# hliangzhao/torch-on-k8s

Hardware: AMD Instinct MI355X
Metric: tokens_per_s (higher is better)
Workload: dtype bf16; 1 GPU; model=llama3-8b, global_batch=8, seq_len=4096, parallelism=dp1, attn_impl=hip

## Files before the change

torch_on_k8s_amd/ops/csrc/attention.hip:

```cpp
#include "common.h"

namespace {

using bf16x8v = __attribute__((ext_vector_type(8))) __bf16;
using f32x4 = __attribute__((ext_vector_type(4))) float;

constexpr int BN = 64;
constexpr int NW = 8;
constexpr int NTHREADS = NW * WAVE;
constexpr int BM = NW * 16;
constexpr float NEG_INF = -INFINITY;

DEVINL int swz_off(int row, int row_bytes, int byte_in_row) {
  return (row * row_bytes + byte_in_row) ^ ((row & 15) << 4);
}

DEVINL bf16x8v as_frag(uint4 raw) {
  union { uint4 u; bf16x8v f; } c;
  c.u = raw;
  return c.f;
}

template <int D, int NTH = NTHREADS>
struct TileStage {
// ... 20 lines not shown
      const int vi = threadIdx.x + i * NTH;
      const int row = vi / VPR, cv = vi % VPR;
      *(uint4*)(lds + swz_off(row, D * 2, cv * 16)) = vals[i];
    }
  }

};

template <int D, int NTH = NTHREADS>
struct TileStageT {
  static constexpr int VPR = 64 / 8;
  static constexpr int VPT = D * VPR / NTH;
  uint4 vals[VPT];

  DEVINL void issue(const bf16_t* plane, int col0, long S_pad) {
#pragma unroll
    for (int i = 0; i < VPT; ++i) {
      const int vi = threadIdx.x + i * NTH;
      const int row = vi / VPR, cv = vi % VPR;
      vals[i] = *(const uint4*)(plane + (long)row * S_pad + col0 + cv * 8);
    }
  }

  DEVINL void write(char* lds) const {
#pragma unroll
    for (int i = 0; i < VPT; ++i) {
      const int vi = threadIdx.x + i * NTH;
      const int row = vi / VPR, cv = vi % VPR;
      *(uint4*)(lds + swz_off(row, 128, cv * 16)) = vals[i];
    }
  }
};

template <int RB>
DEVINL bf16x8v read_bfrag(const char* lds, int row, int col_elem) {
  return as_frag(*(const uint4*)(lds + swz_off(row, RB, col_elem * 2)));
}

template <int D>
DEVINL void load_afrags(bf16x8v* frag, const bf16_t* src, long row,
                        long row_limit, long tok_stride, int lane) {
  constexpr int DC = D / 32;
#pragma unroll
  for (int c = 0; c < DC; ++c) {
    uint4 raw = {0, 0, 0, 0};
    if (row < row_limit)
      raw = *(const uint4*)(src + row * tok_stride + c * 32 + (lane >> 4) * 8);
    frag[c] = as_frag(raw);
  }
}

using f32x16 = __attribute__((ext_vector_type(16))) float;

DEVINL uint32_t pack_bf16(float lo, float hi) {
  return (uint32_t)f2bfbits(lo) | ((uint32_t)f2bfbits(hi) << 16);
}

template <int D, bool CAUSAL>
__global__ __launch_bounds__(NTHREADS) void attn_fwd_kernel_v3(
    const bf16_t* __restrict__ q, const bf16_t* __restrict__ k,
    const bf16_t* __restrict__ vt, bf16_t* __restrict__ o,
    float* __restrict__ lse, int B, int S, int Hq, int Hkv, int S_pad,
    float scale) {
  constexpr int QC = D / 16;
  constexpr int DT = D / 32;
  constexpr int BM3 = NW * 32;
  constexpr int KB = BN * D * 2;
  __shared__ __attribute__((aligned(16))) char smem[2 * (2 * KB)];

  const int lane = threadIdx.x & 63;
  const int hi = lane >> 5;
  const int wid = threadIdx.x >> 6;
  const int m0 = blockIdx.x * BM3;
  const int m0w = m0 + wid * 32;
  const int hq = blockIdx.y;
  const int b = blockIdx.z;
  const int hkv = hq / (Hq / Hkv);

  const long q_tok = (long)Hq * D, kv_tok = (long)Hkv * D;
  const bf16_t* qp = q + ((long)b * S * q_tok) + (long)hq * D;
  const bf16_t* kp = k + ((long)b * S * kv_tok) + (long)hkv * D;
  const bf16_t* vtp = vt + ((long)b * Hkv + hkv) * D * (long)S_pad;
  bf16_t* op = o + ((long)b * S * q_tok) + (long)hq * D;
  float* lsep = lse + ((long)b * Hq + hq) * S;

  const int qrow = m0w + (lane & 31);
  bf16x8v q_reg[QC];
#pragma unroll
  for (int c = 0; c < QC; ++c) {
    uint4 raw = {0, 0, 0, 0};
    if (qrow < S)
      raw = *(const uint4*)(qp + (long)qrow * q_tok + c * 16 + hi * 8);
    q_reg[c] = as_frag(raw);
  }

  f32x16 o_acc[DT];
#pragma unroll
  for (int t = 0; t < DT; ++t)
#pragma unroll
    for (int r = 0; r < 16; ++r) o_acc[t][r] = 0.f;
  float m_run = NEG_INF, l_run = 0.f;

  TileStage<D> k_st;
  TileStageT<D> v_st;
  const int n_end = CAUSAL ? min(S, m0 + BM3) : S;
  k_st.issue(kp, 0, S, kv_tok);
  v_st.issue(vtp, 0, S_pad);
  k_st.write_rm(smem);
// ... 97 lines not shown
              pack_bf16(st[ks][2], st[ks][3]),
              pack_bf16(st[ks][6], st[ks][7]), false, false);
          f0.w[0] = sA[0]; f0.w[1] = sB[0]; f0.w[2] = sA[1]; f0.w[3] = sB[1];
        }
        {
          auto sC = __builtin_amdgcn_permlane32_swap(
              pack_bf16(st[ks][8], st[ks][9]),
              pack_bf16(st[ks][12], st[ks][13]), false, false);
          auto sD = __builtin_amdgcn_permlane32_swap(
              pack_bf16(st[ks][10], st[ks][11]),
              pack_bf16(st[ks][14], st[ks][15]), false, false);
          f1.w[0] = sC[0]; f1.w[1] = sD[0]; f1.w[2] = sC[1]; f1.w[3] = sD[1];
        }
        pa[2 * ks] = f0.f;
        pa[2 * ks + 1] = f1.f;
      }

      __builtin_amdgcn_s_setprio(1);
#pragma unroll
      for (int ks = 0; ks < 4; ++ks)
#pragma unroll
        for (int t = 0; t < DT; ++t) {
          bf16x8v vb = read_bfrag<128>(
              vt_lds, t * 32 + (lane & 31), ks * 16 + hi * 8);
          o_acc[t] = __builtin_amdgcn_mfma_f32_32x32x16_bf16(
              pa[ks], vb, o_acc[t], 0, 0, 0);
        }
      __builtin_amdgcn_s_setprio(0);
    }
    if (more) {
      char* nk = smem + (cur ^ 1) * (2 * KB);
      k_st.write_rm(nk);
      v_st.write(nk + KB);
    }
    __syncthreads();
    cur ^= 1;
  }

#pragma unroll
  for (int r = 0; r < 16; ++r) {
    const int rowidx = (r & 3) + 8 * (r >> 2) + 4 * hi;
    const float lv = __shfl(l_run, rowidx, 64);
    const float inv_l = (lv > 0.f) ? 1.f / lv : 0.f;
    const int row = m0w + rowidx;
    if (row >= S) continue;
#pragma unroll
    for (int t = 0; t < DT; ++t) {
      const int col = t * 32 + (lane & 31);
      op[(long)row * q_tok + col] = f2bf(o_acc[t][r] * inv_l);
    }
  }
  if (hi == 0 && qrow < S)
    lsep[qrow] = (l_run > 0.f) ? m_run + __logf(l_run) : NEG_INF;
}

constexpr int PRE_ROWS = 64;

template <int D>
__global__ __launch_bounds__(256) void attn_bwd_pre_kernel(
    const bf16_t* __restrict__ dout, const bf16_t* __restrict__ o,
    const float* __restrict__ lse, float* __restrict__ dsum,
    float* __restrict__ rc, int Hq, int S, int S_pad, float sqrt_d) {
  constexpr int GL = D / 8;
  constexpr int RPI = WAVE / GL;
  constexpr int NP = 16 / RPI;
  const int lane = threadIdx.x & 63;
  const int wid = threadIdx.x >> 6;
  const int grp = lane / GL, gl = lane % GL;
  const int h = blockIdx.y;
  const long b = blockIdx.z;
  const int s0 = blockIdx.x * PRE_ROWS + wid * 16;
  const long tok = (long)Hq * D;
  const bf16_t* dp = dout + (b * S) * tok + (long)h * D + gl * 8;
  const bf16_t* op = o + (b * S) * tok + (long)h * D + gl * 8;

  uint4 av[NP], bv[NP];
#pragma unroll
  for (int p = 0; p < NP; ++p) {
    const int s = s0 + p * RPI + grp;
    av[p] = bv[p] = uint4{0, 0, 0, 0};
    if (s < S) {
      av[p] = *(const uint4*)(dp + (long)s * tok);
      bv[p] = *(const uint4*)(op + (long)s * tok);
    }
  }
  float mine = 0.f;
#pragma unroll
  for (int p = 0; p < NP; ++p) {
    const uint16_t* ah = (const uint16_t*)&av[p];
    const uint16_t* bh = (const uint16_t*)&bv[p];
    float acc = 0.f;
#pragma unroll
    for (int j = 0; j < 8; ++j)
      acc = fmaf(bfbits2f(ah[j]), bfbits2f(bh[j]), acc);
#pragma unroll
    for (int off = GL / 2; off > 0; off >>= 1)
      acc += __shfl_xor(acc, off, WAVE);
#pragma unroll
    for (int g = 0; g < RPI; ++g) {
      const float vg = __shfl(acc, g * GL, WAVE);
      if (lane == p * RPI + g) mine = vg;
    }
  }
  if (lane < 16) {
    const int s = s0 + lane;
    if (s < S) dsum[(b * Hq + h) * S + s] = mine;
    if (s < S_pad) {
      float* r = rc + (b * Hq + h) * 2 * S_pad;
      const float l = (s < S) ? lse[(b * Hq + h) * S + s] : NEG_INF;
      r[s] = (l == NEG_INF) ? -1e30f : -l * sqrt_d;
      r[S_pad + s] = (s < S) ? -mine : 0.f;
    }
  }
}

DEVINL void repack_pa(const f32x16& pt, bf16x8v& pa0, bf16x8v& pa1) {
  union { uint32_t w[4]; bf16x8v f; } f0, f1;
  auto sA = __builtin_amdgcn_permlane32_swap(
      pack_bf16(pt[0], pt[1]), pack_bf16(pt[4], pt[5]), false, false);
  auto sB = __builtin_amdgcn_permlane32_swap(
      pack_bf16(pt[2], pt[3]), pack_bf16(pt[6], pt[7]), false, false);
  f0.w[0] = sA[0]; f0.w[1] = sB[0]; f0.w[2] = sA[1]; f0.w[3] = sB[1];
  auto sC = __builtin_amdgcn_permlane32_swap(
      pack_bf16(pt[8], pt[9]), pack_bf16(pt[12], pt[13]), false, false);
  auto sD = __builtin_amdgcn_permlane32_swap(
      pack_bf16(pt[10], pt[11]), pack_bf16(pt[14], pt[15]), false, false);
  f1.w[0] = sC[0]; f1.w[1] = sD[0]; f1.w[2] = sC[1]; f1.w[3] = sD[1];
  pa0 = f0.f;
  pa1 = f1.f;
}

template <int D, bool CAUSAL>
__global__ __launch_bounds__(NTHREADS) void attn_bwd_dv_kernel(
    const bf16_t* __restrict__ q, const bf16_t* __restrict__ k,
    const bf16_t* __restrict__ dot_t, const bf16_t* __restrict__ dout,
    const float* __restrict__ lse, const float* __restrict__ dsum,
    bf16_t* __restrict__ dv, int B, int S, int Hq, int Hkv, int S_pad,
    float scale) {
  constexpr int QC = D / 16;
  constexpr int DT = D / 32;
  constexpr int NTH = NTHREADS;
  constexpr int BNK = NW * 32;
  constexpr int KB = BN * D * 2;
  __shared__ __attribute__((aligned(16))) char smem[2 * (2 * KB)];

  const int lane = threadIdx.x & 63;
  const int hi = lane >> 5;
  const int wid = threadIdx.x >> 6;
  const int n0 = blockIdx.x * BNK;
  const int n0w = n0 + wid * 32;
  const int hkv = blockIdx.y;
  const int b = blockIdx.z;
  const int rep = Hq / Hkv;

  const long q_tok = (long)Hq * D, kv_tok = (long)Hkv * D;
  const bf16_t* kp = k + ((long)b * S * kv_tok) + (long)hkv * D;
  bf16_t* dvp = dv + ((long)b * S * kv_tok) + (long)hkv * D;

  const int kvrow = n0w + (lane & 31);
  bf16x8v k_reg[QC];
#pragma unroll
  for (int c = 0; c < QC; ++c) {
    uint4 kr = {0, 0, 0, 0};
    if (kvrow < S)
      kr = *(const uint4*)(kp + (long)kvrow * kv_tok + c * 16 + hi * 8);
    k_reg[c] = as_frag(kr);
  }

  f32x16 dv_acc[DT];
#pragma unroll
  for (int t = 0; t < DT; ++t)
#pragma unroll
    for (int r = 0; r < 16; ++r) dv_acc[t][r] = 0.f;

  const int m_start = CAUSAL ? (n0 / BN) * BN : 0;
  const long dplane = (long)D * S_pad;
  TileStage<D, NTH> q_st;
  TileStageT<D, NTH> do_st;
  const bf16_t* dot0 = dot_t + ((long)b * Hq + hkv * rep) * dplane;
  q_st.issue(q + ((long)b * S * q_tok) + (long)(hkv * rep) * D, m_start, S,
             q_tok);
  do_st.issue(dot0, m_start, S_pad);
// ... 437 lines not shown
  constexpr int STB = DkdvStage<D>::BYTES;
  __shared__ __attribute__((aligned(16))) char smem[2 * STB + BNK * D * 2];
  char* v_lds = smem + 2 * STB;

  const int lane = threadIdx.x & 63;
  const int hi = lane >> 5;
  const int wid = threadIdx.x >> 6;
  const int n0 = blockIdx.x * BNK;
  const int n0w = n0 + wid * 64;
  const int hkv = blockIdx.y;
  const int b = blockIdx.z;
  const int rep = Hq / Hkv;

  const long q_tok = (long)Hq * D, kv_tok = (long)Hkv * D;
  const bf16_t* kp = k + ((long)b * S * kv_tok) + (long)hkv * D;
  const bf16_t* vp = v + ((long)b * S * kv_tok) + (long)hkv * D;

  bf16x8v k_reg[2][QC];
#pragma unroll
  for (int hh = 0; hh < 2; ++hh) {
    const int kvrow = n0w + hh * 32 + (lane & 31);
#pragma unroll
    for (int c = 0; c < QC; ++c) {
      uint4 kr = {0, 0, 0, 0};
      if (kvrow < S)
        kr = *(const uint4*)(kp + (long)kvrow * kv_tok + c * 16 + hi * 8);
      k_reg[hh][c] = as_frag(kr);
    }
  }
  {
    constexpr int VPR = D / 8;
#pragma unroll 4
    for (int vi = threadIdx.x; vi < BNK * VPR; vi += NTH_KV) {
      const int row = vi / VPR, cv = vi % VPR;
      uint4 val = {0, 0, 0, 0};
      if (n0 + row < S)
        val = *(const uint4*)(vp + (long)(n0 + row) * kv_tok + cv * 8);
      *(uint4*)(v_lds + swz_off(row, D * 2, cv * 16)) = val;
    }
  }

  f32x16 dk_acc[2][DT], dv_acc[2][DT];
#pragma unroll
  for (int hh = 0; hh < 2; ++hh)
#pragma unroll
    for (int t = 0; t < DT; ++t)
#pragma unroll
      for (int r = 0; r < 16; ++r) {
        dk_acc[hh][t][r] = 0.f;
        dv_acc[hh][t][r] = 0.f;
      }

  const int m_start = CAUSAL ? n0 : 0;
  const float c2 = 1.4426950408889634f * scale;
  const long plane = (long)D * S_pad;
  const long head0 = (long)b * Hq + hkv * rep;
  const bf16_t* qh = q + ((long)b * S * q_tok) + (long)(hkv * rep) * D;
  const bf16_t* doh = dout + ((long)b * S * q_tok) + (long)(hkv * rep) * D;

  DkdvStage<D> stg;
  stg.init(S_pad);
  stg.issue(qh, doh, q_t + head0 * plane, dot_t + head0 * plane,
            rc + head0 * 2 * S_pad, m_start, S, q_tok, S_pad, smem);
  stg.finish();
  __syncthreads();
  int cur = 0;

  for (int g = 0; g < rep; ++g) {
    for (int m0 = m_start; m0 < S; m0 += QROWS) {
      const char* st = smem + cur * STB;
      char* nst = smem + (cur ^ 1) * STB;
      int gn = g, mn = m0 + QROWS;
      if (mn >= S) {
        gn = g + 1;
        mn = m_start;
      }
      const bool more = gn < rep;
      const bool live0 = n0w < S && (!CAUSAL || m0 + QROWS > n0w);
      const bool live1 =
          n0w + 32 < S && (!CAUSAL || m0 + QROWS > n0w + 32);

      if (more)
        stg.issue(qh + (long)gn * D, doh + (long)gn * D,
                  q_t + (head0 + gn) * plane, dot_t + (head0 + gn) * plane,
                  rc + (head0 + gn) * 2 * S_pad, mn, S, q_tok, S_pad, nst);
      f32x16 sv[2], dpv[2];
      if (live1) {
        dkdv_tile_sdp<D, 2>(st, v_lds, k_reg, sv, dpv, wid * 64, lane, hi);
        dkdv_tile_acc<D, CAUSAL, 2>(st, sv, dpv, dk_acc, dv_acc, m0, n0w, S,
                                    lane, hi, c2);
      } else if (live0) {
        dkdv_tile_sdp<D, 1>(st, v_lds, k_reg, sv, dpv, wid * 64, lane, hi);
        dkdv_tile_acc<D, CAUSAL, 1>(st, sv, dpv, dk_acc, dv_acc, m0, n0w, S,
                                    lane, hi, c2);
      }
      if (more) stg.finish();
      __syncthreads();
      cur ^= 1;
    }
  }

  bf16_t* dkp = dk + ((long)b * S * kv_tok) + (long)hkv * D;
  bf16_t* dvp = dv + ((long)b * S * kv_tok) + (long)hkv * D;
#pragma unroll
  for (int hh = 0; hh < 2; ++hh)
#pragma unroll
    for (int r = 0; r < 16; ++r) {
// ... 5 lines not shown
        dkp[off] = f2bf(dk_acc[hh][t][r] * scale);
        dvp[off] = f2bf(dv_acc[hh][t][r]);
      }
    }
}

template <int D, bool CAUSAL>
__global__ __launch_bounds__(NTHREADS) void attn_bwd_dq_kernel(
    const bf16_t* __restrict__ q, const bf16_t* __restrict__ k,
    const bf16_t* __restrict__ v, const bf16_t* __restrict__ dout,
    const bf16_t* __restrict__ k_t, const float* __restrict__ lse,
    const float* __restrict__ dsum, bf16_t* __restrict__ dq, int B, int S,
    int Hq, int Hkv, int S_pad, float scale) {
  constexpr int QC = D / 16;
  constexpr int DT = D / 32;
  constexpr int BM3 = NW * 32;
  constexpr int KB = BN * D * 2;
  __shared__ __attribute__((aligned(16))) char smem[2 * (3 * KB)];

  const int lane = threadIdx.x & 63;
  const int hi = lane >> 5;
  const int wid = threadIdx.x >> 6;
  const int m0 =
      (CAUSAL ? (int)(gridDim.x - 1 - blockIdx.x) : (int)blockIdx.x) * BM3;
  const int m0w = m0 + wid * 32;
  const int hq = blockIdx.y;
  const int b = blockIdx.z;
  const int hkv = hq / (Hq / Hkv);

  const long q_tok = (long)Hq * D, kv_tok = (long)Hkv * D;
  const bf16_t* qp = q + ((long)b * S * q_tok) + (long)hq * D;
  const bf16_t* kp = k + ((long)b * S * kv_tok) + (long)hkv * D;
  const bf16_t* vp = v + ((long)b * S * kv_tok) + (long)hkv * D;
  const bf16_t* dop = dout + ((long)b * S * q_tok) + (long)hq * D;
  const bf16_t* ktp = k_t + ((long)b * Hkv + hkv) * (long)D * S_pad;
  const float* lsep = lse + ((long)b * Hq + hq) * S;
  const float* dsp = dsum + ((long)b * Hq + hq) * S;
  bf16_t* dqp = dq + ((long)b * S * q_tok) + (long)hq * D;

  const int qrow = m0w + (lane & 31);
  bf16x8v q_reg[QC], do_reg[QC];
#pragma unroll
  for (int c = 0; c < QC; ++c) {
    uint4 qr = {0, 0, 0, 0}, dor = {0, 0, 0, 0};
    if (qrow < S) {
      qr = *(const uint4*)(qp + (long)qrow * q_tok + c * 16 + hi * 8);
      dor = *(const uint4*)(dop + (long)qrow * q_tok + c * 16 + hi * 8);
    }
    q_reg[c] = as_frag(qr);
    do_reg[c] = as_frag(dor);
  }
  const float lse_lane = (qrow < S) ? lsep[qrow] : NEG_INF;
  const float ds_lane = (qrow < S) ? dsp[qrow] : 0.f;

  f32x16 dq_acc[DT];
#pragma unroll
  for (int t = 0; t < DT; ++t)
#pragma unroll
    for (int r = 0; r < 16; ++r) dq_acc[t][r] = 0.f;

  TileStage<D> k_st, v_st;
  TileStageT<D> kt_st;
  const int n_end = CAUSAL ? min(S, m0 + BM3) : S;
  k_st.issue(kp, 0, S, kv_tok);
  v_st.issue(vp, 0, S, kv_tok);
  kt_st.issue(ktp, 0, S_pad);
  k_st.write_rm(smem);
  kt_st.write(smem + KB);
  v_st.write_rm(smem + 2 * KB);
  __syncthreads();
  int cur = 0;

  for (int n0 = 0; n0 < n_end; n0 += BN) {
    char* k_lds = smem + cur * (3 * KB);
    char* kt_lds = k_lds + KB;
    char* v_lds = k_lds + 2 * KB;
    const bool more = n0 + BN < n_end;
    if (more) {
      k_st.issue(kp, n0 + BN, S, kv_tok);
      v_st.issue(vp, n0 + BN, S, kv_tok);
      kt_st.issue(ktp, n0 + BN, S_pad);
    }

    const bool strip_live = !CAUSAL || (n0 <= m0w + 31);
    if (strip_live) {
#pragma unroll
      for (int ks = 0; ks < 2; ++ks) {
        f32x16 sv, dpv;
#pragma unroll
        for (int r = 0; r < 16; ++r) {
          sv[r] = 0.f;
          dpv[r] = 0.f;
        }
#pragma unroll
        for (int c = 0; c < QC; ++c) {
          bf16x8v ka = read_bfrag<D * 2>(
              k_lds, ks * 32 + (lane & 31), c * 16 + hi * 8);
          sv = __builtin_amdgcn_mfma_f32_32x32x16_bf16(
              ka, q_reg[c], sv, 0, 0, 0);
          bf16x8v va = read_bfrag<D * 2>(
              v_lds, ks * 32 + (lane & 31), c * 16 + hi * 8);
          dpv = __builtin_amdgcn_mfma_f32_32x32x16_bf16(
              va, do_reg[c], dpv, 0, 0, 0);
        }

        f32x16 dst;
        const bool need_mask = (CAUSAL && n0 + ks * 32 + 32 > m0w) ||
                               (n0 + ks * 32 + 32 > S) || (m0w + 32 > S);
#pragma unroll
        for (int r = 0; r < 16; ++r) {
          float pv = __expf(sv[r] * scale - lse_lane);
          if (need_mask) {
            const int kvg = n0 + ks * 32 + (r & 3) + 8 * (r >> 2) + 4 * hi;
            if (!(qrow < S && kvg < S && (!CAUSAL || kvg <= qrow) &&
                  lse_lane != NEG_INF))
              pv = 0.f;
          }
          dst[r] = pv * (dpv[r] - ds_lane);
        }

        bf16x8v da0, da1;
        {
          union { uint32_t w[4]; bf16x8v f; } f0, f1;
          auto sA = __builtin_amdgcn_permlane32_swap(
              pack_bf16(dst[0], dst[1]), pack_bf16(dst[4], dst[5]), false,
              false);
          auto sB = __builtin_amdgcn_permlane32_swap(
              pack_bf16(dst[2], dst[3]), pack_bf16(dst[6], dst[7]), false,
              false);
          f0.w[0] = sA[0]; f0.w[1] = sB[0]; f0.w[2] = sA[1]; f0.w[3] = sB[1];
          auto sC = __builtin_amdgcn_permlane32_swap(
              pack_bf16(dst[8], dst[9]), pack_bf16(dst[12], dst[13]), false,
              false);
          auto sD = __builtin_amdgcn_permlane32_swap(
              pack_bf16(dst[10], dst[11]), pack_bf16(dst[14], dst[15]),
              false, false);
          f1.w[0] = sC[0]; f1.w[1] = sD[0]; f1.w[2] = sC[1]; f1.w[3] = sD[1];
          da0 = f0.f;
          da1 = f1.f;
        }
#pragma unroll
        for (int t = 0; t < DT; ++t) {
          bf16x8v b0 = read_bfrag<128>(
              kt_lds, t * 32 + (lane & 31), ks * 32 + hi * 8);
          dq_acc[t] = __builtin_amdgcn_mfma_f32_32x32x16_bf16(
              da0, b0, dq_acc[t], 0, 0, 0);
          bf16x8v b1 = read_bfrag<128>(
              kt_lds, t * 32 + (lane & 31), ks * 32 + 16 + hi * 8);
          dq_acc[t] = __builtin_amdgcn_mfma_f32_32x32x16_bf16(
              da1, b1, dq_acc[t], 0, 0, 0);
        }
      }
    }
    if (more) {
      char* nk = smem + (cur ^ 1) * (3 * KB);
      k_st.write_rm(nk);
      kt_st.write(nk + KB);
      v_st.write_rm(nk + 2 * KB);
    }
    __syncthreads();
    cur ^= 1;
  }

#pragma unroll
  for (int r = 0; r < 16; ++r) {
    const int row = m0w + (r & 3) + 8 * (r >> 2) + 4 * hi;
    if (row >= S) continue;
#pragma unroll
    for (int t = 0; t < DT; ++t) {
      const int col = t * 32 + (lane & 31);
      dqp[(long)row * q_tok + col] = f2bf(dq_acc[t][r] * scale);
    }
  }
}

}

extern "C" {

hipError_t tok_attn_fwd(const void* q, const void* k, const void* vt, void* o,
                        float* lse, int B, int S, int Hq, int Hkv, int D,
                        int S_pad, int causal, hipStream_t stream) {
  dim3 grid((S + NW * 32 - 1) / (NW * 32), Hq, B);
  const float scale = 1.f / sqrtf((float)D);
#define LAUNCH_FWD(DD, CC)                                                    \
  attn_fwd_kernel_v3<DD, CC><<<grid, NTHREADS, 0, stream>>>(                  \
      (const bf16_t*)q, (const bf16_t*)k, (const bf16_t*)vt, (bf16_t*)o,     \
      lse, B, S, Hq, Hkv, S_pad, scale)
  if (D == 128) { if (causal) LAUNCH_FWD(128, true); else LAUNCH_FWD(128, false); }
  else if (D == 64) { if (causal) LAUNCH_FWD(64, true); else LAUNCH_FWD(64, false); }
  else return hipErrorInvalidValue;
#undef LAUNCH_FWD
  return hipGetLastError();
}

hipError_t tok_attn_bwd(const void* q, const void* k, const void* v,
                        const void* o, const void* dout, const void* q_t,
                        const void* k_t, const void* dot_t, const float* lse,
                        float* dsum_ws, float* rc_ws, void* dq, void* dk,
                        void* dv, int B, int S, int Hq, int Hkv, int D,
                        int S_pad, int causal, hipStream_t stream, int split) {
  const float scale = 1.f / sqrtf((float)D);
  dim3 gpre((S + PRE_ROWS - 1) / PRE_ROWS, Hq, B);
  if (D == 128)
    attn_bwd_pre_kernel<128><<<gpre, 256, 0, stream>>>(
        (const bf16_t*)dout, (const bf16_t*)o, lse, dsum_ws, rc_ws, Hq, S,
        S_pad, 1.f / scale);
  else if (D == 64)
    attn_bwd_pre_kernel<64><<<gpre, 256, 0, stream>>>(
        (const bf16_t*)dout, (const bf16_t*)o, lse, dsum_ws, rc_ws, Hq, S,
        S_pad, 1.f / scale);
  else
    return hipErrorInvalidValue;

  dim3 gkv((S + NW * 32 - 1) / (NW * 32), Hkv, B);
  dim3 gkvf((S + NW_KV * 64 - 1) / (NW_KV * 64), Hkv, B);
  dim3 gq((S + NW * 32 - 1) / (NW * 32), Hq, B);
#define LAUNCH_BWD(DD, CC)                                                    \
  do {                                                                        \
    if (split) {                                                              \
      attn_bwd_dv_kernel<DD, CC><<<gkv, NTHREADS, 0, stream>>>(               \
          (const bf16_t*)q, (const bf16_t*)k, (const bf16_t*)dot_t,           \
          (const bf16_t*)dout, lse, dsum_ws, (bf16_t*)dv, B, S, Hq, Hkv,     \
          S_pad, scale);                                                      \
      attn_bwd_dk_kernel<DD, CC><<<gkv, NTHREADS, 0, stream>>>(               \
          (const bf16_t*)q, (const bf16_t*)k, (const bf16_t*)v,               \
          (const bf16_t*)dout, (const bf16_t*)q_t, lse, dsum_ws,              \
          (bf16_t*)dk, B, S, Hq, Hkv, S_pad, scale);                          \
    } else {                                                                  \
      attn_bwd_dkdv_kernel<DD, CC><<<gkvf, NTH_KV, 0, stream>>>(              \
          (const bf16_t*)q, (const bf16_t*)k, (const bf16_t*)v,               \
          (const bf16_t*)dout, (const bf16_t*)q_t, (const bf16_t*)dot_t,      \
          rc_ws, (bf16_t*)dk, (bf16_t*)dv, B, S, Hq, Hkv, S_pad, scale);      \
    }                                                                         \
    attn_bwd_dq_kernel<DD, CC><<<gq, NTHREADS, 0, stream>>>(                  \
        (const bf16_t*)q, (const bf16_t*)k, (const bf16_t*)v,                 \
        (const bf16_t*)dout, (const bf16_t*)k_t, lse, dsum_ws, (bf16_t*)dq,  \
        B, S, Hq, Hkv, S_pad, scale);                                         \
  } while (0)
  if (D == 128) { if (causal) LAUNCH_BWD(128, true); else LAUNCH_BWD(128, false); }
  else { if (causal) LAUNCH_BWD(64, true); else LAUNCH_BWD(64, false); }
// ... 5 lines not shown
```

torch_on_k8s_amd/ops/csrc/bindings.cpp:

```cpp
#include <torch/extension.h>
#include <ATen/hip/impl/HIPStreamMasqueradingAsCUDA.h>
#include <hip/hip_runtime.h>

extern "C" {
hipError_t tok_rmsnorm_fwd(const void* x, const void* w, void* y, float* invr,
                           long nrows, int H, float eps, hipStream_t stream);
int tok_rmsnorm_dw_rsplit(long nrows, int H);
hipError_t tok_rmsnorm_bwd(const void* x, const void* w, const void* dy,
                           const float* invr, void* dx, float* dw_f32,
                           float* dw_ws, long nrows, int H,
                           hipStream_t stream);
hipError_t tok_rmsnorm_res_fwd(const void* x, const void* res, const void* w,
                               void* xr, void* y, float* invr, long nrows,
                               int H, float eps, hipStream_t stream);
hipError_t tok_rmsnorm_res_bwd(const void* xr, const void* w, const void* dy,
                               const void* dxr_in, const float* invr,
                               void* dx, float* dw_f32, float* dw_ws,
                               long nrows, int H, hipStream_t stream);
hipError_t tok_swiglu_fwd(const void* gu, void* out, long rows, int I,
                          hipStream_t stream);
hipError_t tok_swiglu_bwd(const void* dout, const void* gu, void* dgu,
                          long rows, int I, hipStream_t stream);
hipError_t tok_qkv_rope_fwd(const void* qkv, void* q, void* k, void* v,
                            const float* cos_tab, const float* sin_tab,
                            long tokens, int Hq, int Hkv, int D,
                            long table_rows, hipStream_t stream);
hipError_t tok_qkv_rope_bwd(const void* dq, const void* dk, const void* dv,
                            void* dqkv, const float* cos_tab,
                            const float* sin_tab, long tokens, int Hq,
                            int Hkv, int D, long table_rows,
                            hipStream_t stream);
hipError_t tok_rope(const void* x, void* y, const float* cos_tab,
                    const float* sin_tab, long rows_total, int heads, int D,
                    long table_rows, float sign, hipStream_t stream);
hipError_t tok_adamw(void* p, const void* g, float* m, float* v, long n,
                     float lr, float beta1, float beta2, float eps, float wd,
                     int step, float gscale, const int* step_dev,
                     const float* lr_dev, const float* gscale_dev,
                     hipStream_t stream);
int tok_grad_sumsq_max_blocks();
int tok_grad_sumsq_blocks(long n);
hipError_t tok_grad_sumsq(const void* g, long n, float* partials, int nblocks,
                          hipStream_t stream);
hipError_t tok_grad_norm_finalize(const float* partials, long count,
                                  float inv_count, float clip, float* out,
                                  hipStream_t stream);
hipError_t tok_mfma_probe_16x16x32(const void* A, const void* B, float* D,
                                   hipStream_t stream);
hipError_t tok_mfma_probe_32x32x16(const void* A, const void* B, float* D,
                                   hipStream_t stream);
hipError_t tok_attn_fwd(const void* q, const void* k, const void* vt, void* o,
                        float* lse, int B, int S, int Hq, int Hkv, int D,
                        int S_pad, int causal, hipStream_t stream);
hipError_t tok_attn_bwd(const void* q, const void* k, const void* v,
                        const void* o, const void* dout, const void* q_t,
                        const void* k_t, const void* dot_t, const float* lse,
                        float* dsum_ws, float* rc_ws, void* dq, void* dk,
                        void* dv, int B, int S, int Hq, int Hkv, int D,
                        int S_pad, int causal, hipStream_t stream, int split);
hipError_t tok_transpose_head(const void* in, void* out, int B, int S, int H,
                              int D, int S_pad, hipStream_t stream);
hipError_t tok_attn_decode(const void* q, const void* k, const void* v,
                           void* out, int B, int T, const int* T_dev,
                           int Tmax, int Hq, int Hkv, int D,
                           hipStream_t stream);
hipError_t tok_layernorm_fwd(const void* x, const void* w, const void* b,
                             void* y, float* mu, float* rstd, long nrows,
                             int H, float eps, hipStream_t stream);
hipError_t tok_layernorm_bwd(const void* x, const void* w, const void* dy,
                             const float* mu, const float* rstd, void* dx,
                             float* dw, float* db, long nrows, int H,
                             hipStream_t stream);
hipError_t tok_ce_fwd(const void* logits, const int* labels, float* loss,
                      float* lse, long rows, int V, hipStream_t stream);
hipError_t tok_ce_bwd(const void* logits, const int* labels, const float* lse,
                      const float* gscale, void* dlogits, long rows, int V,
                      hipStream_t stream);
}

namespace {

#define CHECK_BF16_CUDA(t)                                                    \
  TORCH_CHECK(t.is_cuda(), #t " must be on GPU");                             \
  TORCH_CHECK(t.scalar_type() == at::kBFloat16, #t " must be bf16");          \
  TORCH_CHECK(t.is_contiguous(), #t " must be contiguous")

#define TOK_HIP_OK(expr)                                                      \
  do {                                                                        \
    hipError_t _e = (expr);                                                   \
    TORCH_CHECK(_e == hipSuccess, "HIP kernel launch failed: ",               \
                hipGetErrorString(_e));                                       \
  } while (0)

hipStream_t current_stream() {
  return at::hip::getCurrentHIPStreamMasqueradingAsCUDA().stream();
}

std::vector<at::Tensor> rmsnorm_fwd(at::Tensor x, at::Tensor w, double eps) {
  CHECK_BF16_CUDA(x);
  CHECK_BF16_CUDA(w);
  const long H = x.size(-1);
  TORCH_CHECK(H % 8 == 0, "hidden dim must be a multiple of 8");
  TORCH_CHECK(w.numel() == H, "weight shape mismatch");
  const long nrows = x.numel() / H;
  auto y = at::empty_like(x);
  auto invr = at::empty({nrows}, x.options().dtype(at::kFloat));
// ... 173 lines not shown
  CHECK_BF16_CUDA(p);
  CHECK_BF16_CUDA(g);
  TORCH_CHECK(m.scalar_type() == at::kFloat && v.scalar_type() == at::kFloat);
  const long n = p.numel();
  TORCH_CHECK(n % 8 == 0, "bucket size must be a multiple of 8");
  TORCH_CHECK(g.numel() == n && m.numel() == n && v.numel() == n);
  const int* sd = nullptr;
  if (step_dev.has_value()) {
    TORCH_CHECK(step_dev->scalar_type() == at::kInt && step_dev->is_cuda());
    sd = step_dev->data_ptr<int>();
  }
  const float* lrd = dev_f32_scalar(lr_dev, "lr_dev");
  const float* gsd = dev_f32_scalar(gscale_dev, "gscale_dev");
  TOK_HIP_OK(tok_adamw(p.data_ptr(), g.data_ptr(), m.data_ptr<float>(),
                       v.data_ptr<float>(), n, (float)lr, (float)beta1,
                       (float)beta2, (float)eps, (float)wd, (int)step,
                       (float)gscale, sd, lrd, gsd, current_stream()));
}

long grad_sumsq_blocks(long n) { return tok_grad_sumsq_blocks(n); }

long grad_sumsq_max_blocks() { return tok_grad_sumsq_max_blocks(); }

void grad_sumsq_(at::Tensor g, at::Tensor partials) {
  CHECK_BF16_CUDA(g);
  TORCH_CHECK(partials.is_cuda() && partials.scalar_type() == at::kFloat &&
                  partials.is_contiguous(),
              "partials must be a contiguous fp32 GPU tensor");
  const long n = g.numel();
  TORCH_CHECK(n % 8 == 0, "bucket size must be a multiple of 8");
  const long nb = partials.numel();
  TORCH_CHECK(nb >= 1 && nb <= tok_grad_sumsq_max_blocks(),
              "partials must hold 1..", tok_grad_sumsq_max_blocks(),
              " slots (use grad_sumsq_blocks(n))");
  TOK_HIP_OK(tok_grad_sumsq(g.data_ptr(), n, partials.data_ptr<float>(),
                            (int)nb, current_stream()));
}

void grad_norm_finalize_(at::Tensor partials, at::Tensor out, double inv_count,
                         double clip) {
  TORCH_CHECK(partials.is_cuda() && partials.scalar_type() == at::kFloat &&
                  partials.is_contiguous(),
              "partials must be a contiguous fp32 GPU tensor");
  TORCH_CHECK(out.is_cuda() && out.scalar_type() == at::kFloat &&
                  out.is_contiguous() && out.numel() >= 2,
              "out must be a contiguous fp32 GPU tensor of >= 2 elements");
  TOK_HIP_OK(tok_grad_norm_finalize(partials.data_ptr<float>(),
                                    partials.numel(), (float)inv_count,
                                    (float)clip, out.data_ptr<float>(),
                                    current_stream()));
}

std::vector<at::Tensor> attn_fwd(at::Tensor q, at::Tensor k, at::Tensor v,
                                 bool causal) {
  CHECK_BF16_CUDA(q);
  CHECK_BF16_CUDA(k);
  CHECK_BF16_CUDA(v);
  const int B = q.size(0), S = q.size(1), Hq = q.size(2), D = q.size(3);
  const int Hkv = k.size(2);
  TORCH_CHECK(D == 128 || D == 64, "head_dim must be 64 or 128");
  TORCH_CHECK(Hq % Hkv == 0, "GQA requires Hq % Hkv == 0");
  TORCH_CHECK(k.sizes() == v.sizes() && k.size(0) == B && k.size(1) == S);
  auto o = at::empty_like(q);
  auto lse = at::empty({B, Hq, S}, q.options().dtype(at::kFloat));
  const int S_pad = (S + 63) / 64 * 64;
  auto vt = at::empty({B, Hkv, D, S_pad}, q.options());
  TOK_HIP_OK(tok_transpose_head(v.data_ptr(), vt.data_ptr(), B, S, Hkv, D,
                                S_pad, current_stream()));
  TOK_HIP_OK(tok_attn_fwd(q.data_ptr(), k.data_ptr(), vt.data_ptr(),
                          o.data_ptr(), lse.data_ptr<float>(), B, S, Hq, Hkv,
                          D, S_pad, causal ? 1 : 0, current_stream()));
  return {o, lse};
}

std::vector<at::Tensor> attn_bwd(at::Tensor q, at::Tensor k, at::Tensor v,
                                 at::Tensor o, at::Tensor lse, at::Tensor dout,
                                 bool causal, bool split) {
  CHECK_BF16_CUDA(q);
  CHECK_BF16_CUDA(dout);
  const int B = q.size(0), S = q.size(1), Hq = q.size(2), D = q.size(3);
  const int Hkv = k.size(2);
  auto dq = at::empty_like(q);
  auto dk = at::empty_like(k);
  auto dv = at::empty_like(v);
  auto dsum = at::empty({B, Hq, S}, q.options().dtype(at::kFloat));
  const int S_pad = (S + 63) / 64 * 64;
  auto rc = at::empty({B, Hq, 2, S_pad}, q.options().dtype(at::kFloat));
  auto qt = at::empty({B, Hq, D, S_pad}, q.options());
  auto kt = at::empty({B, Hkv, D, S_pad}, q.options());
  auto dot = at::empty({B, Hq, D, S_pad}, q.options());
  TOK_HIP_OK(tok_transpose_head(q.data_ptr(), qt.data_ptr(), B, S, Hq, D,
                                S_pad, current_stream()));
  TOK_HIP_OK(tok_transpose_head(k.data_ptr(), kt.data_ptr(), B, S, Hkv, D,
                                S_pad, current_stream()));
  TOK_HIP_OK(tok_transpose_head(dout.data_ptr(), dot.data_ptr(), B, S, Hq, D,
                                S_pad, current_stream()));
  TOK_HIP_OK(tok_attn_bwd(q.data_ptr(), k.data_ptr(), v.data_ptr(),
                          o.data_ptr(), dout.data_ptr(), qt.data_ptr(),
                          kt.data_ptr(), dot.data_ptr(),
                          lse.data_ptr<float>(), dsum.data_ptr<float>(),
                          rc.data_ptr<float>(), dq.data_ptr(), dk.data_ptr(), dv.data_ptr(), B, S,
                          Hq, Hkv, D, S_pad, causal ? 1 : 0, current_stream(),
                          split ? 1 : 0));
  return {dq, dk, dv};
}

at::Tensor attn_decode(at::Tensor q, at::Tensor kcache, at::Tensor vcache,
                       long T, c10::optional<at::Tensor> T_dev) {
  CHECK_BF16_CUDA(q);
  CHECK_BF16_CUDA(kcache);
  CHECK_BF16_CUDA(vcache);
  const int B = q.size(0), Hq = q.size(1), D = q.size(2);
  const int Tmax = kcache.size(1), Hkv = kcache.size(2);
  TORCH_CHECK(T_dev.has_value() || (T >= 1 && T <= Tmax));
  TORCH_CHECK(D == 64 || D == 128);
  const int* td = nullptr;
  if (T_dev.has_value()) {
    TORCH_CHECK(T_dev->scalar_type() == at::kInt && T_dev->is_cuda());
    td = T_dev->data_ptr<int>();
  }
  auto out = at::empty_like(q);
  TOK_HIP_OK(tok_attn_decode(q.data_ptr(), kcache.data_ptr(),
                             vcache.data_ptr(), out.data_ptr(), B, (int)T,
                             td, Tmax, Hq, Hkv, D, current_stream()));
// ... 36 lines not shown
}

std::vector<at::Tensor> ce_fwd(at::Tensor logits, at::Tensor labels) {
  CHECK_BF16_CUDA(logits);
  TORCH_CHECK(labels.scalar_type() == at::kInt && labels.is_cuda());
  const long V = logits.size(-1);
  TORCH_CHECK(V % 8 == 0, "vocab must be a multiple of 8");
  const long rows = logits.numel() / V;
  TORCH_CHECK(labels.numel() == rows);
  auto loss = at::empty({rows}, logits.options().dtype(at::kFloat));
  auto lse = at::empty({rows}, logits.options().dtype(at::kFloat));
  TOK_HIP_OK(tok_ce_fwd(logits.data_ptr(), labels.data_ptr<int>(),
                        loss.data_ptr<float>(), lse.data_ptr<float>(), rows,
                        (int)V, current_stream()));
  return {loss, lse};
}

at::Tensor ce_bwd(at::Tensor logits, at::Tensor labels, at::Tensor lse,
                  at::Tensor gscale) {
  CHECK_BF16_CUDA(logits);
  TORCH_CHECK(gscale.scalar_type() == at::kFloat && gscale.is_cuda());
  const long V = logits.size(-1);
  const long rows = logits.numel() / V;
  auto dlogits = at::empty_like(logits);
  TOK_HIP_OK(tok_ce_bwd(logits.data_ptr(), labels.data_ptr<int>(),
                        lse.data_ptr<float>(), gscale.data_ptr<float>(),
                        dlogits.data_ptr(), rows, (int)V, current_stream()));
  return dlogits;
}

at::Tensor mfma_probe(at::Tensor A, at::Tensor B) {
  CHECK_BF16_CUDA(A);
  CHECK_BF16_CUDA(B);
  if (A.size(0) == 16) {
    TORCH_CHECK(A.sizes() == at::IntArrayRef({16, 32}) &&
                B.sizes() == at::IntArrayRef({32, 16}));
    auto D = at::empty({16, 16}, A.options().dtype(at::kFloat));
    TOK_HIP_OK(tok_mfma_probe_16x16x32(A.data_ptr(), B.data_ptr(),
                                       D.data_ptr<float>(), current_stream()));
    return D;
  }
  TORCH_CHECK(A.sizes() == at::IntArrayRef({32, 16}) &&
              B.sizes() == at::IntArrayRef({16, 32}));
  auto D = at::empty({32, 32}, A.options().dtype(at::kFloat));
  TOK_HIP_OK(tok_mfma_probe_32x32x16(A.data_ptr(), B.data_ptr(),
                                     D.data_ptr<float>(), current_stream()));
  return D;
}

}

PYBIND11_MODULE(TORCH_EXTENSION_NAME, mod) {
  mod.def("mfma_probe", &mfma_probe, "MFMA 16x16x32 bf16 layout probe");
  mod.def("attn_fwd", &attn_fwd, "Flash attention forward (bf16, gfx950)");
  mod.def("attn_bwd", &attn_bwd, "Flash attention backward (bf16, gfx950)",
          py::arg("q"), py::arg("k"), py::arg("v"), py::arg("o"),
          py::arg("lse"), py::arg("dout"), py::arg("causal"),
          py::arg("split") = false);
  mod.def("ce_fwd", &ce_fwd, "Fused cross-entropy forward (bf16, gfx950)");
  mod.def("layernorm_fwd", &layernorm_fwd, "LayerNorm forward (bf16, gfx950)");
  mod.def("attn_decode", &attn_decode,
          "Single-token KV-cache attention decode (bf16, gfx950)",
          py::arg("q"), py::arg("kcache"), py::arg("vcache"), py::arg("T"),
          py::arg("T_dev") = py::none());
  mod.def("layernorm_bwd", &layernorm_bwd, "LayerNorm backward (bf16, gfx950)");
  mod.def("ce_bwd", &ce_bwd, "Fused cross-entropy backward (bf16, gfx950)");
  mod.def("rmsnorm_fwd", &rmsnorm_fwd, "RMSNorm forward (bf16, gfx950)");
  mod.def("rmsnorm_bwd", &rmsnorm_bwd, "RMSNorm backward (bf16, gfx950)");
  mod.def("rmsnorm_res_fwd", &rmsnorm_res_fwd,
          "Fused residual-add + RMSNorm forward (bf16, gfx950)",
          py::arg("x"), py::arg("res"), py::arg("w"), py::arg("eps"));
  mod.def("rmsnorm_res_bwd", &rmsnorm_res_bwd,
          "Fused residual-add + RMSNorm backward (bf16, gfx950)",
          py::arg("xr"), py::arg("w"), py::arg("dy"), py::arg("dxr"),
          py::arg("invr"));
  mod.def("swiglu_fwd", &swiglu_fwd,
          "Fused SwiGLU over packed gate_up (bf16, gfx950)");
  mod.def("swiglu_bwd", &swiglu_bwd,
          "Fused SwiGLU backward (bf16, gfx950)");
  mod.def("qkv_rope_fwd", &qkv_rope_fwd,
          "Packed-QKV split + RoPE (bf16, gfx950)");
  mod.def("qkv_rope_bwd", &qkv_rope_bwd,
          "Packed-QKV gather + inverse RoPE (bf16, gfx950)");
  mod.def("rope", &rope, "Rotary embedding rotate-half (bf16, gfx950)");
  mod.def("adamw_", &adamw_, "Fused AdamW on a flat bucket (gfx950)",
          py::arg("p"), py::arg("g"), py::arg("m"), py::arg("v"),
          py::arg("lr"), py::arg("beta1"), py::arg("beta2"), py::arg("eps"),
          py::arg("wd"), py::arg("step"), py::arg("gscale"),
          py::arg("step_dev") = py::none(), py::arg("lr_dev") = py::none(),
          py::arg("gscale_dev") = py::none());
  mod.def("grad_sumsq_blocks", &grad_sumsq_blocks,
          "Partial slots grad_sumsq_ needs for a bucket of n elements");
  mod.def("grad_sumsq_max_blocks", &grad_sumsq_max_blocks,
          "Grid cap of grad_sumsq_");
  mod.def("grad_sumsq_", &grad_sumsq_,
          "Per-block sum of squares of a flat bf16 bucket (gfx950)");
  mod.def("grad_norm_finalize_", &grad_norm_finalize_,
          "Sum partials -> {norm, clip-folded grad scale} (gfx950)",
          py::arg("partials"), py::arg("out"), py::arg("inv_count"),
          py::arg("clip"));
}
```

Baseline: 18940 tokens/s.

## Add v4 flash-attention forward with lazy rescaling, exp2 softmax, and LDS-staged output

Adds a new forward attention kernel, used by default, that works in the log2 domain with fused FMA+exp2. It defers the online-softmax rescale unless the running max rises past a threshold, adds scheduling hints and priority around the MFMA blocks, and stages the normalized output through shared memory so global stores are coalesced 16-byte writes. It also switches bf16 packing to a vector convert and uses exp2 in the dq backward kernel. The goal is fewer exp/rescale operations and cheaper output writes, at the cost of subtle numerical differences and more complex scheduling.

```diff
diff --git a/torch_on_k8s_amd/ops/csrc/attention.hip b/torch_on_k8s_amd/ops/csrc/attention.hip
--- a/torch_on_k8s_amd/ops/csrc/attention.hip
+++ b/torch_on_k8s_amd/ops/csrc/attention.hip
@@ -96,8 +96,30 @@
 
 using f32x16 = __attribute__((ext_vector_type(16))) float;
 
+using f32x2 = __attribute__((ext_vector_type(2))) float;
+using bf16x2v = __attribute__((ext_vector_type(2))) __bf16;
+
 DEVINL uint32_t pack_bf16(float lo, float hi) {
-  return (uint32_t)f2bfbits(lo) | ((uint32_t)f2bfbits(hi) << 16);
+  const f32x2 f = {lo, hi};
+  union { bf16x2v b; uint32_t u; } c;
+  c.b = __builtin_convertvector(f, bf16x2v);
+  return c.u;
+}
+
+DEVINL void repack_pa(const f32x16& pt, bf16x8v& pa0, bf16x8v& pa1) {
+  union { uint32_t w[4]; bf16x8v f; } f0, f1;
+  auto sA = __builtin_amdgcn_permlane32_swap(
+      pack_bf16(pt[0], pt[1]), pack_bf16(pt[4], pt[5]), false, false);
+  auto sB = __builtin_amdgcn_permlane32_swap(
+      pack_bf16(pt[2], pt[3]), pack_bf16(pt[6], pt[7]), false, false);
+  f0.w[0] = sA[0]; f0.w[1] = sB[0]; f0.w[2] = sA[1]; f0.w[3] = sB[1];
+  auto sC = __builtin_amdgcn_permlane32_swap(
+      pack_bf16(pt[8], pt[9]), pack_bf16(pt[12], pt[13]), false, false);
+  auto sD = __builtin_amdgcn_permlane32_swap(
+      pack_bf16(pt[10], pt[11]), pack_bf16(pt[14], pt[15]), false, false);
+  f1.w[0] = sC[0]; f1.w[1] = sD[0]; f1.w[2] = sC[1]; f1.w[3] = sD[1];
+  pa0 = f0.f;
+  pa1 = f1.f;
 }
 
 template <int D, bool CAUSAL>
@@ -301,6 +323,217 @@
   }
   if (hi == 0 && qrow < S)
     lsep[qrow] = (l_run > 0.f) ? m_run + __logf(l_run) : NEG_INF;
+}
+
+constexpr float LOG2E = 1.4426950408889634f;
+constexpr float LN2 = 0.6931471805599453f;
+
+template <int D, bool CAUSAL>
+__global__ __launch_bounds__(NTHREADS) void attn_fwd_kernel_v4(
+    const bf16_t* __restrict__ q, const bf16_t* __restrict__ k,
+    const bf16_t* __restrict__ vt, bf16_t* __restrict__ o,
+    float* __restrict__ lse, int B, int S, int Hq, int Hkv, int S_pad,
+    float scale) {
+  constexpr int QC = D / 16;
+  constexpr int DT = D / 32;
+  constexpr int BM3 = NW * 32;
+  constexpr int KB = BN * D * 2;
+  constexpr int OWB = 32 * D * 2;
+  static_assert(NW * OWB <= 2 * (2 * KB), "O staging fits the K|VT buffers");
+  __shared__ __attribute__((aligned(16))) char smem[2 * (2 * KB)];
+
+  const int lane = threadIdx.x & 63;
+  const int hi = lane >> 5;
+  const int wid = threadIdx.x >> 6;
+  const int m0 = blockIdx.x * BM3;
+  const int m0w = m0 + wid * 32;
+  const int hq = blockIdx.y;
+  const int b = blockIdx.z;
+  const int hkv = hq / (Hq / Hkv);
+
+  const long q_tok = (long)Hq * D, kv_tok = (long)Hkv * D;
+  const bf16_t* qp = q + ((long)b * S * q_tok) + (long)hq * D;
+  const bf16_t* kp = k + ((long)b * S * kv_tok) + (long)hkv * D;
+  const bf16_t* vtp = vt + ((long)b * Hkv + hkv) * D * (long)S_pad;
+  bf16_t* op = o + ((long)b * S * q_tok) + (long)hq * D;
+  float* lsep = lse + ((long)b * Hq + hq) * S;
+
+  const int qrow = m0w + (lane & 31);
+  bf16x8v q_reg[QC];
+#pragma unroll
+  for (int c = 0; c < QC; ++c) {
+    uint4 raw = {0, 0, 0, 0};
+    if (qrow < S)
+      raw = *(const uint4*)(qp + (long)qrow * q_tok + c * 16 + hi * 8);
+    q_reg[c] = as_frag(raw);
+  }
+
+  f32x16 o_acc[DT];
+#pragma unroll
+  for (int t = 0; t < DT; ++t)
+#pragma unroll
+    for (int r = 0; r < 16; ++r) o_acc[t][r] = 0.f;
+  float m_run = NEG_INF, l_run = 0.f;
+  const float c2 = scale * LOG2E;
+
+  TileStage<D> k_st;
+  TileStageT<D> v_st;
+  const int n_end = CAUSAL ? min(S, m0 + BM3) : S;
+  k_st.issue(kp, 0, S, kv_tok);
+  v_st.issue(vtp, 0, S_pad);
+  k_st.write_rm(smem);
+  v_st.write(smem + KB);
+  __syncthreads();
+  int cur = 0;
+
+  for (int n0 = 0; n0 < n_end; n0 += BN) {
+    char* k_lds = smem + cur * (2 * KB);
+    char* vt_lds = k_lds + KB;
+    const bool more = n0 + BN < n_end;
+    if (more) {
+      k_st.issue(kp, n0 + BN, S, kv_tok);
+      v_st.issue(vtp, n0 + BN, S_pad);
+    }
+
+    const bool strip_live = !CAUSAL || (n0 <= m0w + 31);
+    if (strip_live) {
+      f32x16 st[2];
+#pragma unroll
+      for (int ks = 0; ks < 2; ++ks)
+#pragma unroll
+        for (int r = 0; r < 16; ++r) st[ks][r] = 0.f;
+      __builtin_amdgcn_s_setprio(1);
+      bf16x8v ka[2][QC];
+#pragma unroll
+      for (int ks = 0; ks < 2; ++ks)
+#pragma unroll
+        for (int c = 0; c < QC; ++c)
+          ka[ks][c] = read_bfrag<D * 2>(
+              k_lds, ks * 32 + (lane & 31), c * 16 + hi * 8);
+#pragma unroll
+      for (int ks = 0; ks < 2; ++ks)
+#pragma unroll
+        for (int c = 0; c < QC; ++c)
+          st[ks] = __builtin_amdgcn_mfma_f32_32x32x16_bf16(
+              ka[ks][c], q_reg[c], st[ks], 0, 0, 0);
+      __builtin_amdgcn_sched_group_barrier(0x100, QC, 0);
+#pragma unroll
+      for (int c = 0; c < QC; ++c) {
+        __builtin_amdgcn_sched_group_barrier(0x008, 1, 0);
+        __builtin_amdgcn_sched_group_barrier(0x100, 1, 0);
+      }
+      __builtin_amdgcn_sched_group_barrier(0x008, QC, 0);
+      __builtin_amdgcn_s_setprio(0);
+
+      const bool needs_mask = (n0 + BN > S) ||
+                              (CAUSAL && (n0 + BN - 1 > m0w));
+      if (needs_mask) {
+#pragma unroll
+        for (int ks = 0; ks < 2; ++ks)
+#pragma unroll
+          for (int r = 0; r < 16; ++r) {
+            const int kvg = n0 + ks * 32 + (r & 3) + 8 * (r >> 2) + 4 * hi;
+            if ((CAUSAL && kvg > qrow) || kvg >= S || qrow >= S)
+              st[ks][r] = NEG_INF;
+          }
+      }
+      float mx = NEG_INF;
+#pragma unroll
+      for (int ks = 0; ks < 2; ++ks)
+#pragma unroll
+        for (int r = 0; r < 16; ++r) mx = fmaxf(mx, st[ks][r]);
+      mx = fmaxf(mx, __shfl_xor(mx, 32, 64)) * c2;
+      constexpr float DEFER_THR = 8.f * LOG2E;
+      const bool rescale = !__all(mx <= m_run + DEFER_THR);
+      float alpha = 1.f;
+      if (rescale) {
+        const float mn = fmaxf(m_run, mx);
+        alpha = (m_run == NEG_INF) ? 0.f
+                                   : __builtin_amdgcn_exp2f(m_run - mn);
+        m_run = mn;
+      }
+      const float neg_m = (m_run == NEG_INF) ? 0.f : -m_run;
+      float rsum = 0.f;
+#pragma unroll
+      for (int ks = 0; ks < 2; ++ks)
+#pragma unroll
+        for (int r = 0; r < 16; ++r) {
+          const float pe =
+              __builtin_amdgcn_exp2f(__builtin_fmaf(st[ks][r], c2, neg_m));
+          st[ks][r] = pe;
+          rsum += pe;
+        }
+      rsum += __shfl_xor(rsum, 32, 64);
+      l_run = l_run * alpha + rsum;
+
+      if (rescale) {
+#pragma unroll
+        for (int r = 0; r < 16; ++r) {
+          const int rowidx = (r & 3) + 8 * (r >> 2) + 4 * hi;
+          const float ar = __shfl(alpha, rowidx, 64);
+#pragma unroll
+          for (int t = 0; t < DT; ++t) o_acc[t][r] *= ar;
+        }
+      }
+
+      bf16x8v pa[4];
+#pragma unroll
+      for (int ks = 0; ks < 2; ++ks)
+        repack_pa(st[ks], pa[2 * ks], pa[2 * ks + 1]);
+
+      __builtin_amdgcn_s_setprio(1);
+#pragma unroll
+      for (int ks = 0; ks < 4; ++ks)
+#pragma unroll
+        for (int t = 0; t < DT; ++t) {
+          bf16x8v vb = read_bfrag<128>(
+              vt_lds, t * 32 + (lane & 31), ks * 16 + hi * 8);
+          o_acc[t] = __builtin_amdgcn_mfma_f32_32x32x16_bf16(
+              pa[ks], vb, o_acc[t], 0, 0, 0);
+        }
+      __builtin_amdgcn_s_setprio(0);
+    }
+    if (more) {
+      char* nk = smem + (cur ^ 1) * (2 * KB);
+      k_st.write_rm(nk);
+      v_st.write(nk + KB);
+    }
+    __syncthreads();
+    cur ^= 1;
+  }
+
+  char* ow = smem + wid * OWB;
+  if (hi == 0)
+    *(float*)(ow + (lane & 31) * 4) = (l_run > 0.f) ? 1.f / l_run : 0.f;
+  f32x4 il[4];
+#pragma unroll
+  for (int g = 0; g < 4; ++g)
+    il[g] = *(const f32x4*)(ow + (8 * g + 4 * hi) * 4);
+  __builtin_amdgcn_wave_barrier();
+#pragma unroll
+  for (int r = 0; r < 16; ++r) {
+    const int rowidx = (r & 3) + 8 * (r >> 2) + 4 * hi;
+#pragma unroll
+    for (int t = 0; t < DT; ++t) {
+      const int cb = (t * 32 + (lane & 31)) * 2;
+      *(bf16_t*)(ow + rowidx * (D * 2) + (cb ^ (hi << 6))) =
+          f2bf(o_acc[t][r] * il[r >> 2][r & 3]);
+    }
+  }
+  __builtin_amdgcn_wave_barrier();
+  constexpr int CPR = D * 2 / 16;
+  constexpr int RPI = WAVE / CPR;
+#pragma unroll
+  for (int i = 0; i < 32 / RPI; ++i) {
+    const int row = i * RPI + lane / CPR;
+    const int ch = lane % CPR;
+    const uint4 val = *(const uint4*)(
+        ow + row * (D * 2) + ((ch * 16) ^ (((row >> 2) & 1) << 6)));
+    if (m0w + row < S)
+      *(uint4*)(op + (long)(m0w + row) * q_tok + ch * 8) = val;
+  }
+  if (hi == 0 && qrow < S)
+    lsep[qrow] = (l_run > 0.f) ? m_run * LN2 + __logf(l_run) : NEG_INF;
 }
 
 constexpr int PRE_ROWS = 64;
@@ -361,22 +594,6 @@
       r[S_pad + s] = (s < S) ? -mine : 0.f;
     }
   }
-}
-
-DEVINL void repack_pa(const f32x16& pt, bf16x8v& pa0, bf16x8v& pa1) {
-  union { uint32_t w[4]; bf16x8v f; } f0, f1;
-  auto sA = __builtin_amdgcn_permlane32_swap(
-      pack_bf16(pt[0], pt[1]), pack_bf16(pt[4], pt[5]), false, false);
-  auto sB = __builtin_amdgcn_permlane32_swap(
-      pack_bf16(pt[2], pt[3]), pack_bf16(pt[6], pt[7]), false, false);
-  f0.w[0] = sA[0]; f0.w[1] = sB[0]; f0.w[2] = sA[1]; f0.w[3] = sB[1];
-  auto sC = __builtin_amdgcn_permlane32_swap(
-      pack_bf16(pt[8], pt[9]), pack_bf16(pt[12], pt[13]), false, false);
-  auto sD = __builtin_amdgcn_permlane32_swap(
-      pack_bf16(pt[10], pt[11]), pack_bf16(pt[14], pt[15]), false, false);
-  f1.w[0] = sC[0]; f1.w[1] = sD[0]; f1.w[2] = sC[1]; f1.w[3] = sD[1];
-  pa0 = f0.f;
-  pa1 = f1.f;
 }
 
 template <int D, bool CAUSAL>
@@ -920,7 +1137,7 @@
       }
 
   const int m_start = CAUSAL ? n0 : 0;
-  const float c2 = 1.4426950408889634f * scale;
+  const float c2 = LOG2E * scale;
   const long plane = (long)D * S_pad;
   const long head0 = (long)b * Hq + hkv * rep;
   const bf16_t* qh = q + ((long)b * S * q_tok) + (long)(hkv * rep) * D;
@@ -1032,6 +1249,8 @@
   }
   const float lse_lane = (qrow < S) ? lsep[qrow] : NEG_INF;
   const float ds_lane = (qrow < S) ? dsp[qrow] : 0.f;
+  const float c2 = scale * LOG2E;
+  const float nl2 = -lse_lane * LOG2E;
 
   f32x16 dq_acc[DT];
 #pragma unroll
@@ -1089,7 +1308,7 @@
                                (n0 + ks * 32 + 32 > S) || (m0w + 32 > S);
 #pragma unroll
         for (int r = 0; r < 16; ++r) {
-          float pv = __expf(sv[r] * scale - lse_lane);
+          float pv = __builtin_amdgcn_exp2f(__builtin_fmaf(sv[r], c2, nl2));
           if (need_mask) {
             const int kvg = n0 + ks * 32 + (r & 3) + 8 * (r >> 2) + 4 * hi;
             if (!(qrow < S && kvg < S && (!CAUSAL || kvg <= qrow) &&
@@ -1100,25 +1319,7 @@
         }
 
         bf16x8v da0, da1;
-        {
-          union { uint32_t w[4]; bf16x8v f; } f0, f1;
-          auto sA = __builtin_amdgcn_permlane32_swap(
-              pack_bf16(dst[0], dst[1]), pack_bf16(dst[4], dst[5]), false,
-              false);
-          auto sB = __builtin_amdgcn_permlane32_swap(
-              pack_bf16(dst[2], dst[3]), pack_bf16(dst[6], dst[7]), false,
-              false);
-          f0.w[0] = sA[0]; f0.w[1] = sB[0]; f0.w[2] = sA[1]; f0.w[3] = sB[1];
-          auto sC = __builtin_amdgcn_permlane32_swap(
-              pack_bf16(dst[8], dst[9]), pack_bf16(dst[12], dst[13]), false,
-              false);
-          auto sD = __builtin_amdgcn_permlane32_swap(
-              pack_bf16(dst[10], dst[11]), pack_bf16(dst[14], dst[15]),
-              false, false);
-          f1.w[0] = sC[0]; f1.w[1] = sD[0]; f1.w[2] = sC[1]; f1.w[3] = sD[1];
-          da0 = f0.f;
-          da1 = f1.f;
-        }
+        repack_pa(dst, da0, da1);
 #pragma unroll
         for (int t = 0; t < DT; ++t) {
           bf16x8v b0 = read_bfrag<128>(
@@ -1160,13 +1361,22 @@
 
 hipError_t tok_attn_fwd(const void* q, const void* k, const void* vt, void* o,
                         float* lse, int B, int S, int Hq, int Hkv, int D,
-                        int S_pad, int causal, hipStream_t stream) {
+                        int S_pad, int causal, hipStream_t stream,
+                        int variant) {
   dim3 grid((S + NW * 32 - 1) / (NW * 32), Hq, B);
   const float scale = 1.f / sqrtf((float)D);
+  if (variant != 0 && variant != 1) return hipErrorInvalidValue;
 #define LAUNCH_FWD(DD, CC)                                                    \
-  attn_fwd_kernel_v3<DD, CC><<<grid, NTHREADS, 0, stream>>>(                  \
-      (const bf16_t*)q, (const bf16_t*)k, (const bf16_t*)vt, (bf16_t*)o,     \
-      lse, B, S, Hq, Hkv, S_pad, scale)
+  do {                                                                        \
+    if (variant == 1)                                                         \
+      attn_fwd_kernel_v3<DD, CC><<<grid, NTHREADS, 0, stream>>>(              \
+          (const bf16_t*)q, (const bf16_t*)k, (const bf16_t*)vt, (bf16_t*)o, \
+          lse, B, S, Hq, Hkv, S_pad, scale);                                  \
+    else                                                                      \
+      attn_fwd_kernel_v4<DD, CC><<<grid, NTHREADS, 0, stream>>>(              \
+          (const bf16_t*)q, (const bf16_t*)k, (const bf16_t*)vt, (bf16_t*)o, \
+          lse, B, S, Hq, Hkv, S_pad, scale);                                  \
+  } while (0)
   if (D == 128) { if (causal) LAUNCH_FWD(128, true); else LAUNCH_FWD(128, false); }
   else if (D == 64) { if (causal) LAUNCH_FWD(64, true); else LAUNCH_FWD(64, false); }
   else return hipErrorInvalidValue;
diff --git a/torch_on_k8s_amd/ops/csrc/bindings.cpp b/torch_on_k8s_amd/ops/csrc/bindings.cpp
--- a/torch_on_k8s_amd/ops/csrc/bindings.cpp
+++ b/torch_on_k8s_amd/ops/csrc/bindings.cpp
@@ -51,7 +51,8 @@
                                    hipStream_t stream);
 hipError_t tok_attn_fwd(const void* q, const void* k, const void* vt, void* o,
                         float* lse, int B, int S, int Hq, int Hkv, int D,
-                        int S_pad, int causal, hipStream_t stream);
+                        int S_pad, int causal, hipStream_t stream,
+                        int variant);
 hipError_t tok_attn_bwd(const void* q, const void* k, const void* v,
                         const void* o, const void* dout, const void* q_t,
                         const void* k_t, const void* dot_t, const float* lse,
@@ -331,7 +332,7 @@
 }
 
 std::vector<at::Tensor> attn_fwd(at::Tensor q, at::Tensor k, at::Tensor v,
-                                 bool causal) {
+                                 bool causal, int64_t variant) {
   CHECK_BF16_CUDA(q);
   CHECK_BF16_CUDA(k);
   CHECK_BF16_CUDA(v);
@@ -340,6 +341,7 @@
   TORCH_CHECK(D == 128 || D == 64, "head_dim must be 64 or 128");
   TORCH_CHECK(Hq % Hkv == 0, "GQA requires Hq % Hkv == 0");
   TORCH_CHECK(k.sizes() == v.sizes() && k.size(0) == B && k.size(1) == S);
+  TORCH_CHECK(variant == 0 || variant == 1, "attn_fwd variant must be 0 or 1");
   auto o = at::empty_like(q);
   auto lse = at::empty({B, Hq, S}, q.options().dtype(at::kFloat));
   const int S_pad = (S + 63) / 64 * 64;
@@ -348,7 +350,8 @@
                                 S_pad, current_stream()));
   TOK_HIP_OK(tok_attn_fwd(q.data_ptr(), k.data_ptr(), vt.data_ptr(),
                           o.data_ptr(), lse.data_ptr<float>(), B, S, Hq, Hkv,
-                          D, S_pad, causal ? 1 : 0, current_stream()));
+                          D, S_pad, causal ? 1 : 0, current_stream(),
+                          (int)variant));
   return {o, lse};
 }
 
@@ -491,7 +494,9 @@
 
 PYBIND11_MODULE(TORCH_EXTENSION_NAME, mod) {
   mod.def("mfma_probe", &mfma_probe, "MFMA 16x16x32 bf16 layout probe");
-  mod.def("attn_fwd", &attn_fwd, "Flash attention forward (bf16, gfx950)");
+  mod.def("attn_fwd", &attn_fwd, "Flash attention forward (bf16, gfx950)",
+          py::arg("q"), py::arg("k"), py::arg("v"), py::arg("causal"),
+          py::arg("variant") = 0);
   mod.def("attn_bwd", &attn_bwd, "Flash attention backward (bf16, gfx950)",
           py::arg("q"), py::arg("k"), py::arg("v"), py::arg("o"),
           py::arg("lse"), py::arg("dout"), py::arg("causal"),
```

New measurement: 19420 tokens/s, median of 6. 1.03x the previous value.
